# rileyhales/river-route

Measured on AMD Instinct MI355X. Metric: reach-steps/sec, higher is better.
Workload: dtype f64

## Files before the change

river_route_amd/csrc/rr_engine.hip:

```cpp
#include "rr_common.hpp"
#include "rr_kernels_tick.hpp"
#include "rr_kernels_tile.hpp"
#include "rr_kernels_uh.hpp"
#include "rr_kernels_rec.hpp"
#include "rr_kernels_runoff.hpp"
#include "rr_kernels_direct.hpp"
#include "rr_kernels_metrics.hpp"
#include "rr_kernels_overlap.hpp"
#include "rr_kernels_adjoint.hpp"
#include "rr_kernels_adjoint_unit.hpp"
#include "rr_exec.hpp"


extern "C" {

int rr_version(void) { return RR_VERSION_NUM; }

const char *rr_last_error(void) { return g_err.c_str(); }

int rr_device_count(void)
{
    int c = 0;
    if (hipGetDeviceCount(&c) != hipSuccess) return 0;
    return c;
// ... 10 lines not shown
        if (P->ev_last) (void)hipEventDestroy(P->ev_last);
    }
    delete P;
}

int rr_plan_create(int64_t n, const int32_t *csc_indptr, const int32_t *csc_indices, int device, rr_plan **out)
{
    if (!out) return fail(RR_E_INVALID, "rr_plan_create: null out");
    *out = nullptr;
    rr_plan *P = new (std::nothrow) rr_plan();
    if (!P) return fail(RR_E_ALLOC, "rr_plan_create: out of memory");
    if (const char *e = getenv("RR_HW_INPASS")) P->hw_inpass = atoi(e) != 0;
    if (const char *e = getenv("RR_ALLOC_FAIL_AT")) rr::g_dev_fail_in = std::max(0, atoi(e));
    if (const char *e = getenv("RR_WAVE")) { P->wave_enabled = atoi(e) != 0; P->wave_forced = atoi(e) == 1; }
    if (const char *e = getenv("RR_REC_BATCHES")) { P->rec_batches = std::max(1, std::min(kRecMaxLaunchBatches, atoi(e))); P->rec_batches_forced = true; }
    if (const char *e = getenv("RR_WAVE_K")) P->wave_K = std::max(kRec, atoi(e) / kRec * kRec);
    std::string err;
    int rc = rr::build_host_plan(n, csc_indptr, csc_indices, P->h, err);
    if (rc) { delete P; return fail(rc, err); }
    if (device != RR_DEVICE_NONE) {
        int count = rr_device_count(), cus = 0;
        if (device >= 0 && device < count && hipDeviceGetAttribute(&cus, hipDeviceAttributeMultiprocessorCount, device) == hipSuccess && cus > 0) P->cu_count = cus;
    }
    {
        P->wave_threads = kTileThreads;
        int32_t block = P->wave_threads;
        if (const char *e = getenv("RR_TILE_BLOCK")) block = std::max(8, std::min(block, atoi(e)));
        std::vector<int32_t> lag_of((size_t)n);
        for (int64_t i = 0; i < n; ++i) lag_of[i] = P->h.lag[P->h.inv[i]];
        rr::build_tile_plan(P->h.down, lag_of, block, P->tp);
        if (const char *e = getenv("RR_DIRECT")) P->direct_enabled = atoi(e) != 0;
        P->direct_block = block;
        rr::build_direct_plan(P->h.down, lag_of, std::min<int32_t>(kDirectLanes, block), kDirectMaxWindow - 2, block, P->dp);
        P->direct_window = 3;
        for (int32_t sp : P->dp.tile_span) P->direct_window = std::max(P->direct_window, sp + 3);
    }
    if (device != RR_DEVICE_NONE) {
        int count = rr_device_count();
        if (device < 0 || device >= count) {
            delete P;
            return fail(RR_E_NO_DEVICE, "rr_plan_create: HIP device " + std::to_string(device) + " not available (" +
                                            std::to_string(count) + " visible)");
        }
        hipError_t e = hipSetDevice(device);
        if (e != hipSuccess) { delete P; return fail(RR_E_HIP, hipGetErrorString(e)); }
        P->device = device;
        {
            size_t free_b = 0, total_b = 0;
            if (hipMemGetInfo(&free_b, &total_b) == hipSuccess) P->dev_total_bytes = total_b;
        }
        if (const char *e2 = getenv("RR_TILE_LEAN")) P->lean_enabled = atoi(e2) != 0;
        for (int v = 0; v < 7; ++v)
            if (hipFuncSetAttribute((const void *)tile_kernel(v < 4 ? (v & 1) != 0 : v == 5, v < 4 && (v & 2) != 0, v >= 4, v == 6), hipFuncAttributeMaxDynamicSharedMemorySize,
                                    (int)tile_lds_bytes(P->wave_threads)) != hipSuccess) {
                (void)hipGetLastError();
                P->wave_enabled = false;
            }
        for (int v = 0; v < 4; ++v)
            if (hipFuncSetAttribute((const void *)tile_ens_kernel((v & 1) != 0, v >= 2), hipFuncAttributeMaxDynamicSharedMemorySize, (int)tile_lds_bytes(kTileThreads)) != hipSuccess) {
                (void)hipGetLastError();
                P->ens_enabled = false;
            }
        if (const char *e2 = getenv("RR_UH_PAIRS")) P->uh_pairs = atoi(e2) != 0;
        for (int v = 0; v < 4; ++v)
            (void)hipFuncSetAttribute((const void *)rec_in_uh_kernel((v & 1) != 0, 64, 1 + (v >> 1)), hipFuncAttributeMaxDynamicSharedMemorySize, (int)rec_in_uh_lds_bytes(64, 1 + (v >> 1)));
        (void)hipGetLastError();
        const rr::HostPlan &H = P->h;
        const int64_t ni = (int64_t)H.inner_pos.size();
        rc = P->d_child_ptr.alloc(n + 1);
        for (DevBuf<int32_t> *col : {&P->d_lag, &P->d_perm, &P->d_inv}) if (!rc) rc = col->alloc(n);
        if (!rc) rc = P->d_inner_pos.alloc(ni);
        if (!rc) rc = P->d_hwc.alloc(n);
        if (!rc) rc = P->d_bidx.alloc(n);
        if (!rc) rc = P->d_c4_params.alloc(n);
        if (!rc && P->tp.ok) {
            const rr::TilePlan &TP = P->tp;
            const int64_t np = TP.np;
            std::vector<int32_t> inner_idx;
            inner_idx.reserve(ni);
            for (int64_t i = 0; i < n; ++i) if (H.child_ptr[H.inv[i] + 1] > H.child_ptr[H.inv[i]]) inner_idx.push_back((int32_t)i);
            rc = assign(P->d_inner_idx, inner_idx);
            if (!rc) rc = upload_tile_meta(P, TP.lag, TP.xpos, TP.tile_flags);
            if (!rc) rc = assign(P->ts.perm, TP.perm);
            if (!rc) rc = assign(P->d_tinv, TP.inv);
            for (DevBuf<double> *coef : {&P->ts.coef, &P->d_coef_unit, &P->d_coef_hw}) if (!rc) rc = coef->alloc(3 * np);
            if (!rc) rc = P->d_hwcoef.alloc(3 * n);
            if (!rc) rc = P->d_hwq.alloc(n);
            for (DevBuf<double> *state : {&P->ts.sq, &P->ts.ss, &P->ts.si, &P->ts.sqch}) if (!rc) rc = state->alloc(np);
            if (!rc) rc = P->d_full.alloc(n);
            if (!rc) rc = P->d_chan.alloc(n);
        }
        if (!rc) rc = upload_direct_plan(P);
        for (DevBuf<double> *row : {&P->d_w, &P->d_c1row_h, &P->d_c2, &P->d_c3, &P->d_c4}) if (!rc) rc = row->alloc(n);
        if (!rc) rc = P->d_x.alloc(3 * n);
        if (!rc) rc = P->d_isum.alloc(n);
        if (!rc) rc = P->d_qch.alloc(n);
        if (!rc) rc = dev_upload(P->d_child_ptr, H.child_ptr);
        if (!rc) rc = dev_upload(P->d_lag, H.lag);
        if (!rc) rc = dev_upload(P->d_perm, H.perm);
        if (!rc) rc = dev_upload(P->d_inv, H.inv);
        if (!rc) rc = dev_upload(P->d_inner_pos, H.inner_pos);
        if (!rc) rc = dev_upload(P->d_hwc, H.hw_children);
        if (rc) { rr_plan_destroy(P); return rc; }
    }
    *out = P;
    return RR_OK;
}
// ... 1690 lines not shown
```

river_route_amd/csrc/rr_exec.hpp:

```cpp
#pragma once

#include <atomic>

#include "rr_devbuf.hpp"

using rr::DevBuf;


enum class Mode { Rapid, Muskingum, Unit };

struct Rows {
    const double *dev_in = nullptr;
    const float *dev_in32 = nullptr;
    const double *host_in = nullptr;
    int64_t rows_in = 0;
    double *dev_out = nullptr;
    double *host_out = nullptr;
    int64_t rows_out = 0;
    float *dev_out32 = nullptr;
    int64_t out_factor = 1;
    const double *uh_kernel = nullptr, *uh_state = nullptr;
    int64_t uh_nks = 0;
    const RunoffArgs *runoff = nullptr;
    int64_t members = 0, in_pitch = 0, out_pitch = 0;
// ... 612 lines not shown
        if (io.uh_kernel || io.runoff || (!io.dev_out && !io.dev_out32) || (mode == Mode::Unit && (io.dev_in32 || P->n_ghost > 0 || P->n_export > 0)) || nsub > kDirectMaxSub ||
            (io.dev_out32 && (io.out_factor < 1 || (S.KC * kRec) % io.out_factor != 0 || T % io.out_factor != 0)))
            return fail(RR_E_STATE, "route: the direct row path was chosen for a call it does not take");
        const rr::TilePlan &TP = P->dp.skel;
        const int64_t K = S.KC * kRec;
        S.n_tasks = (S.T + K - 1) / K;
        S.n_diags = TP.n_tiles > 0 ? S.n_macro + TP.n_levels - 1 : 0;
        S.n_in_batches = (S.total + 14) / kRecRows + 1;
        S.n_out_batches = TP.np > 0 ? (S.total + kRecRows - 1) / kRecRows : 0;
        for (int32_t i : P->export_reach) {
            if (!P->dp.big[i]) { S.export_lanes = true; continue; }
            S.export_skel = true;
            const int32_t p = TP.inv[i];
            S.export_skew = std::max<int64_t>(S.export_skew, (int64_t)TP.tile_level[TP.tile_of[p]] * S.KS * kRec + (TP.lag[p] & kLagMask));
        }
        DirectArgs &da = S.da;
        da.tiles = P->d_dtiles; da.n_tiles = P->dp.n_tiles; da.lane = P->d_dlane; da.coef = P->d_dcoef; da.q = P->d_dq; da.qch = nullptr;
        if (mode == Mode::Unit) { da.q = P->d_full; da.qch = P->d_chan; }
        da.send_ptr = P->d_dsend_ptr; da.send_lane = P->d_dsend_lane;
        da.in = S.has_in ? io.dev_in : nullptr; da.out = io.dev_out; da.n = n; da.in_rows = (uint32_t)std::max<int64_t>(1, io.rows_in); da.out_rows = (uint32_t)std::max<int64_t>(1, io.rows_out);
        da.in32 = S.has_in ? io.dev_in32 : nullptr; da.out32 = io.dev_out32; da.factor = (int32_t)std::max<int64_t>(1, io.out_factor);
        da.nsub = (int32_t)nsub; da.inv_nsub = 1.0 / (double)nsub;
        da.in32_sel = P->in32_big_endian ? kSelSwap : kSelNative; da.out32_sel = P->out32_big_endian ? kSelSwap : kSelNative;
        da.rec = P->d_ring; da.rec_chunks = (uint32_t)std::max<int64_t>(1, S.rec_chunks); da.np = (int32_t)TP.np;
        da.K = (int32_t)K; da.total = (int32_t)S.T;
        da.exports = export_series; da.n_export = (int32_t)P->n_export;
    }
    if (S.kernel == Kernel::Tile) {
        const rr::TilePlan &TP = P->tp;
        const int64_t K = S.KC * kRec;
        S.n_diags = S.n_macro + TP.n_levels - 1;
        S.n_in_batches = (S.total + 14) / kRecRows + 1;
        S.n_out_batches = (S.total + kRecRows - 1) / kRecRows;
        S.ghost_slack = P->ghost_reach.empty() ? 0 : S.total_ticks + (int64_t)TP.n_levels * K;
        for (int32_t i : P->ghost_reach) { const int32_t p = TP.inv[i]; S.ghost_slack = std::min<int64_t>(S.ghost_slack, (int64_t)TP.tile_level[TP.tile_of[p]] * K + (TP.lag[p] & kLagMask)); }
        for (int32_t i : P->export_reach) { const int32_t p = TP.inv[i]; S.export_skew = std::max<int64_t>(S.export_skew, (int64_t)TP.tile_level[TP.tile_of[p]] * K + (TP.lag[p] & kLagMask)); }
        S.hw = P->hw_inpass && P->lean_enabled && nsub == 1 && S.members == 0 &&
               (mode == Mode::Unit || (mode == Mode::Rapid && !io.runoff && !io.uh_kernel));
        if (S.members > 0) {
            if (S.members > P->ens_cap || (S.rec_chunks * kRec * TP.np) * S.members > P->d_ring.count()) return fail(RR_E_STATE, "route: the ensemble was not reserved");
            if (io.member_coeffs && S.members > P->mc_sets) return fail(RR_E_STATE, "route: fewer coefficient sets than members");
            S.ring_stride = S.rec_chunks * kRec * TP.np;
            S.ta.sq = P->d_esq; S.ta.ss = P->d_ess; S.ta.si = P->d_esi; S.ta.sqch = nullptr;
        }
    }
    if (getenv("RR_VERBOSE") && S.kernel == Kernel::Direct)
        fprintf(stderr, "rr: n=%lld T=%lld direct rows: K=%lld tiles=%d window=%d holes=%lld outlets=%lld; skeleton: positions=%lld tiles=%d levels=%d ring_chunks=%lld (%.1f GB)\n",
                (long long)n, (long long)T, (long long)(S.KC * kRec), P->dp.n_tiles, P->direct_window, (long long)P->dp.n_holes, (long long)P->dp.n_exports,
                (long long)P->dp.skel.np, P->dp.skel.n_tiles, P->dp.skel.n_levels, (long long)S.rec_chunks, (double)S.rec_chunks * kRec * P->dp.skel.np * 8 / 1e9);
    else if (getenv("RR_VERBOSE"))
        fprintf(stderr, "rr: n=%lld T=%lld nsub=%lld tiled=%d K=%lld tiles=%d levels=%d block=%d ghosts=%lld ring_chunks=%lld (%.1f GB) rec_batches=%lld lds=%zu hw_inpass=%d (%lld of %lld headwater positions)\n",
                (long long)n, (long long)T, (long long)nsub, (int)(S.kernel == Kernel::Tile), (long long)(S.KC * kRec), P->tp.n_tiles, P->tp.n_levels, P->tp.block,
                (long long)P->tp.n_ghost, (long long)S.rec_chunks, S.kernel == Kernel::Tile ? (double)S.rec_chunks * kRec * P->tp.np * 8 / 1e9 : 0.0,
                (long long)S.rec_nb, tile_lds_bytes(P->wave_threads), (int)S.hw, (long long)(S.hw ? P->hw_counts[0] : 0), (long long)P->hw_counts[1]);
    if (S.kernel == Kernel::Tick) {
        const int64_t lag_rows = (dmax + nsub - 1) / nsub;
        S.ring_rows = S.in_place ? 0 : std::min<int64_t>(T, lag_rows + 2 * C + 2);
        if (S.ring_rows > 0xFFFFFFFFLL || T > 0x7FFFFFFFLL) return fail(RR_E_INVALID, "route: too many time rows");
        if (S.ring_rows * n > P->d_ring.count() || (!S.in_place && C * n > P->d_mrows.count()) || (host_io && C * n > P->d_stage.count()))
            return fail(RR_E_STATE, "route: work rows of the streaming kernel were not reserved");
        TickArgs &a = S.a;
        a.child_ptr = P->d_child_ptr; a.lag = P->d_lag; a.w = P->d_w; a.c2 = P->d_c2; a.c3 = P->d_c3; a.c4 = P->d_c4;
        a.c1row = P->weights_uniform ? P->d_c1row_h : nullptr;
        a.isum = P->d_isum; a.bidx = P->d_bidx;
        a.ghost = ghost_series; a.exports = export_series; a.n_ghost = (int32_t)P->n_ghost; a.n_export = (int32_t)P->n_export;
        a.total_substeps = S.total; a.nsub = Div32((uint32_t)nsub); a.inv_nsub = 1.0 / (double)nsub;
        if (S.in_place) {
            a.in = io.dev_in; a.in_ld = n; a.in_rows = Div32((uint32_t)std::max<int64_t>(1, io.rows_in));
            a.out = io.dev_out; a.out_ld = n; a.out_rows = Div32((uint32_t)io.rows_out);
        } else {
            a.in = S.has_in ? P->d_ring : nullptr; a.in_ld = n; a.in_rows = Div32((uint32_t)S.ring_rows);
            a.out = P->d_ring; a.out_ld = n; a.out_rows = Div32((uint32_t)S.ring_rows);
        }
    }
    S.max_samples = P->sample_every >= kSampleGroup ? (size_t)std::min<int64_t>(4096, S.total_ticks / P->sample_every + 1) : 0;
    if (S.kernel == Kernel::Tile && S.max_samples > 0) S.max_samples = (size_t)std::min<int64_t>(4096, S.n_diags / 4 + 1);
    if (S.kernel == Kernel::Direct && S.max_samples > 0) S.max_samples = (size_t)std::min<int64_t>(4096, S.n_tasks);
    S.max_samples = std::min(S.max_samples, P->ev.size() / 2);
    if (!P->ev_first) return fail(RR_E_STATE, "route: the plan's events were not reserved");
    HIPCHK(hipEventRecord(P->ev_first, stream));
    return RR_OK;
}

int session_begin(rr_plan *P, Mode mode, int64_t T, int64_t nsub, const Rows &io, hipStream_t stream,
                  const double *ghost_series, double *export_series)
{
    if (P->ses.open) return fail(RR_E_STATE, "a routing call is already open on this plan (rr_stream_end it first)");
    const int rc = session_setup(P, mode, T, nsub, io, stream, ghost_series, export_series);
    P->ses.open = rc == RR_OK;
    return rc;
}

void launch_skel_state_out(const TileSet &ks, double *dst, const DevBuf<double> &state, hipStream_t stream)
{
    if (ks.tp->np > 0) hipLaunchKernelGGL(k_skel_state_out, grid1(ks.tp->np), dim3(kBlock), 0, stream, dst, (const double *)state, ks.perm.get(), ks.pmeta.get(), (int32_t)ks.tp->np);
}

void permute_rows_via(rr_plan *P, int which, const RowView &src, const RowView &dst, int64_t t0, int nrows, double *mrows, hipStream_t stream)
{
    const int64_t n = P->h.n;
    constexpr int E = kPermE;
    const int64_t tile = (int64_t)E * kPermThreads;
    const int rpb = (int)std::max<int64_t>(1, P->perm_rows_per_block);
    dim3 g((unsigned)((n + tile - 1) / tile), (unsigned)((nrows + rpb - 1) / rpb));
    const size_t lds_bytes = (size_t)tile * sizeof(double);
    hipLaunchKernelGGL(k_perm_a<E>, g, dim3(kPermThreads), lds_bytes, stream, src, mrows, n,
                       (const uint16_t *)P->d_slot_a[which], (const int32_t *)P->d_m_index[which], t0, nrows, rpb);
// ... 61 lines not shown

int session_launch_tick(rr_plan *P, int64_t tau)
{
    Session &S = P->ses;
    const int64_t n = P->h.n;
    int64_t p_lo, p_hi;
    if (!tick_window(P->h, tau, S.total, p_lo, p_hi)) return RR_OK;
    TickArgs &a = S.a;
    a.p_lo = (int32_t)p_lo; a.p_hi = (int32_t)p_hi; a.tau = tau;
    a.xc = P->d_x + (tau % 3) * n;
    a.xa = P->d_x + ((tau + 2) % 3) * n;
    a.xb = P->d_x + ((tau + 1) % 3) * n;
    const int64_t phase = S.max_samples > 0 ? P->prof_launches % P->sample_every : -1;
    if (phase == 0 && !S.bracket_open && (size_t)P->prof_brackets < S.max_samples) {
        HIPCHK(hipEventRecord(P->ev[2 * P->prof_brackets], S.stream));
        S.bracket_open = true;
    }
    const dim3 g = grid1(p_hi - p_lo);
    const bool one = S.nsub == 1;
    if (S.mode == Mode::Unit) {
        UnitTickArgs ua{};
        ua.t = a; ua.hw_children = P->d_hwc; ua.qch = P->d_qch;
        ua.a2 = P->unit_general ? P->d_a2 : nullptr; ua.c1own = P->d_c1own;
        if (P->unit_general) { ua.t.c1row = nullptr; ua.zc = P->d_z + (tau % 3) * n; ua.za = P->d_z + ((tau + 2) % 3) * n; }
        hipLaunchKernelGGL(tick_unit_kernel(one), g, dim3(kBlock), 0, S.stream, ua);
    } else {
        hipLaunchKernelGGL(tick_kernel(S.mode == Mode::Rapid, one), g, dim3(kBlock), 0, S.stream, a);
    }
    if (S.bracket_open) {
        S.bracket_reaches += p_hi - p_lo;
        ++P->prof_samples;
        if (P->prof_samples % kSampleGroup == 0) {
            HIPCHK(hipEventRecord(P->ev[2 * P->prof_brackets + 1], S.stream));
            ++P->prof_brackets;
            P->ev_reaches.push_back(S.bracket_reaches);
            S.bracket_reaches = 0;
            S.bracket_open = false;
        }
    }
    ++P->prof_launches;
    return RR_OK;
}

typedef void (*tile_kernel_t)(const TileArgs);

constexpr int kTileThreads = 512;
tile_kernel_t tile_kernel(bool unit, bool sub, bool lean = false, bool nolat = false)
{
    constexpr int T = kTileThreads;
    if (lean && nolat && !unit && !sub) return (tile_kernel_t)k_tile<T, false, false, true, true>;
    return unit ? (sub ? (tile_kernel_t)k_tile<T, true, true> : (lean ? (tile_kernel_t)k_tile<T, true, false, true> : (tile_kernel_t)k_tile<T, true, false>))
                : (sub ? (tile_kernel_t)k_tile<T, false, true> : (lean ? (tile_kernel_t)k_tile<T, false, false, true> : (tile_kernel_t)k_tile<T, false, false>));
}

tile_kernel_t tile_ens_kernel(bool sub, bool mcoef = false)
{
    constexpr int T = kTileThreads;
    if (mcoef) return sub ? (tile_kernel_t)k_tile<T, false, true, false, false, true, true> : (tile_kernel_t)k_tile<T, false, false, false, false, true, true>;
    return sub ? (tile_kernel_t)k_tile<T, false, true, false, false, true> : (tile_kernel_t)k_tile<T, false, false, false, false, true>;
}

int launch_tile_diag(rr_plan *P, const TileSet &ts, TileArgs &w, const double *coef_unit, int64_t d, bool sampled)
{
    Session &S = P->ses;
    const rr::TilePlan &TP = *ts.tp;
    const int64_t l_lo = std::max<int64_t>(0, d - (S.n_macro - 1)), l_hi = std::min<int64_t>(TP.n_levels - 1, d);
    if (l_hi < l_lo) return RR_OK;
    int64_t t_lo = TP.level_start[l_lo], t_hi = TP.level_start[l_hi + 1];
    const int64_t K = (int64_t)w.KC * kRec;
    if (l_lo == 0) {
        const int64_t end0 = TP.level_start[1];
        int64_t hi = std::min<int64_t>(t_hi, end0);
        while (hi > t_lo && (d + 1) * K <= TP.tile_lag_lo[hi - 1]) --hi;
        if (t_hi <= end0) t_hi = hi;
    }
    if (t_hi <= t_lo) return RR_OK;
    w.diag = (int32_t)d; w.t_first = (int32_t)t_lo; w.t_last = (int32_t)t_hi - 1;
    const bool sample = sampled && S.max_samples > 0 && (P->prof_launches % 4) == 0 && (size_t)P->prof_brackets < S.max_samples;
    if (sample) HIPCHK(hipEventRecord(P->ev[2 * P->prof_brackets], S.stream));
    const dim3 g((unsigned)std::min<int64_t>(t_hi - t_lo, (int64_t)P->cu_count * (1024 / P->wave_threads)));
    const size_t lds_bytes = tile_lds_bytes(P->wave_threads);
    const bool unit = S.mode == Mode::Unit;
    const bool lean = S.nsub == 1 && P->lean_enabled;
    if (S.members > 0) {
        const dim3 ge((unsigned)std::min<int64_t>(t_hi - t_lo, std::max<int64_t>(1, ((int64_t)P->cu_count * (1024 / kTileThreads) + S.members - 1) / S.members)), (unsigned)S.members);
        const bool mcoef = S.io.member_coeffs;
        w.tile_filter = 0; w.coef = mcoef ? P->d_mcoef.get() : ts.coef.get();
        hipLaunchKernelGGL(tile_ens_kernel(S.nsub > 1, mcoef), ge, dim3((unsigned)kTileThreads), tile_lds_bytes(kTileThreads), S.stream, w);
    } else {
        w.tile_filter = lean ? 1 : 0;
        w.coef = (lean && unit) ? coef_unit : ts.coef.get();
        const int4 *const pos = w.pos;
        if (lean && S.hw) {
            w.pos = P->d_pmeta_hw;
            if (!unit) w.coef = P->d_coef_hw;
        }
        hipLaunchKernelGGL(tile_kernel(unit, S.nsub > 1, lean, S.mode == Mode::Muskingum), g, dim3((unsigned)P->wave_threads), lds_bytes, S.stream, w);
        w.pos = pos;
        if (lean && ts.n_wide > 0) {
            w.tile_filter = 2; w.coef = ts.coef;
            hipLaunchKernelGGL(tile_kernel(unit, false, false), g, dim3((unsigned)P->wave_threads), lds_bytes, S.stream, w);
        }
    }
    if (sample) {
        HIPCHK(hipEventRecord(P->ev[2 * P->prof_brackets + 1], S.stream));
        int64_t moved = 0;
        for (int64_t c = t_lo; c < t_hi; ++c) {
            const int64_t m = d - TP.tile_level[c];
            if (m < 0 || m >= S.n_macro || m * K >= TP.tile_lag_hi[c] + S.total || (m + 1) * K <= TP.tile_lag_lo[c]) continue;
            moved += TP.tile_ptr[c + 1] - TP.tile_ptr[c];
        }
        P->ev_reaches.push_back(moved * K * std::max<int64_t>(1, S.members));
        P->prof_samples += K;
        ++P->prof_brackets;
    }
    return RR_OK;
}

bool tile_diag_launches(const rr_plan *P, const rr::TilePlan &TP, int64_t d)
{
    const Session &S = P->ses;
    const int64_t l_lo = std::max<int64_t>(0, d - (S.n_macro - 1)), l_hi = std::min<int64_t>(TP.n_levels - 1, d);
    return l_hi >= l_lo && TP.level_start[l_hi + 1] > TP.level_start[l_lo];
}

RecPermArgs rec_args(const rr_plan *P, int64_t batch)
{
    const Session &S = P->ses;
    RecPermArgs ra{};
    ra.in32_sel = P->in32_big_endian ? kSelSwap : kSelNative; ra.out32_sel = P->out32_big_endian ? kSelSwap : kSelNative;
    ra.rec = P->d_ring; ra.rec_chunks = Div32((uint32_t)S.rec_chunks); ra.np = tiles_of(P, S.kernel).tp->np;
    ra.T = S.T; ra.total = S.total; ra.batch = batch; ra.nsub = Div32((uint32_t)S.nsub);
    ra.factor = Div32((uint32_t)std::max<int64_t>(1, S.io.out_factor));
    return ra;
}

void launch_ghost_permute(rr_plan *P, int64_t batch)
{
    Session &S = P->ses;
    RecPermArgs ra = rec_args(P, batch);
    ra.T = S.total; ra.nsub = Div32(1u);
    ra.n = P->n_ghost; ra.colmeta = S.kernel == Kernel::Direct ? P->d_kghostmeta : P->d_ghostmeta;
    ra.rows = RowView{const_cast<double *>(S.ghost_series), P->n_ghost, 0, (uint32_t)S.total};
    hipLaunchKernelGGL(k_rec_in<false>, dim3((unsigned)((P->n_ghost + kRecInCols - 1) / kRecInCols)), dim3(kRecInThreads), 0, rec_stream(P), ra);
}

typedef void (*rec_in_uh_t)(const RecPermArgs, const UhArgs);
constexpr int kUhFusedMaxTaps = 64;
int uh_padded_taps(int64_t n_ks) { return n_ks <= 16 ? 16 : (n_ks <= 48 ? 48 : 64); }
rec_in_uh_t rec_in_uh_kernel(bool sub, int64_t n_ks, int batches, bool in32 = false)
// ... 683 lines not shown
```

river_route_amd/csrc/rr_kernels_tile.hpp:

```cpp
#pragma once

namespace {


struct TileMeta {
    int32_t b0, b1;
    int32_t level;
    int32_t lag_lo, lag_hi;
    int32_t flags;
    int32_t pad0, pad1;
};
constexpr int32_t kTileWide = 1, kTileExports = 2, kTaskTested = 4;
struct TileArgs {
    const TileMeta *tiles;
    const int4 *pos;
    const double *coef;
    double *sq, *ss, *si, *sqch;
    double *exports;
    int32_t n_export;
    double *rec;
    Div32 rec_chunks;
    int32_t np, t_first, t_last, KC, diag, n_macro, total, has_lat;
    int32_t tile_filter;
    Div32 nsub;
// ... 8 lines not shown
constexpr uint32_t kBufferFlags = 0x00020000;
constexpr uint32_t kDropAccess = 0xFFFFFFF0u;
typedef unsigned int u32x2 __attribute__((ext_vector_type(2)));
typedef unsigned int u32x4 __attribute__((ext_vector_type(4)));
__device__ __forceinline__ __amdgpu_buffer_rsrc_t make_rsrc(const void *base, uint32_t bytes)
{
    return __builtin_amdgcn_make_buffer_rsrc(const_cast<void *>(base), 0, (int)bytes, (int)kBufferFlags);
}
__device__ __forceinline__ void store_f64(__amdgpu_buffer_rsrc_t r, uint32_t byte_off, double v)
{
    u32x2 bits;
    __builtin_memcpy(&bits, &v, sizeof bits);
    __builtin_amdgcn_raw_buffer_store_b64(bits, r, (int)byte_off, 0, 0);
}
constexpr int kAuxDefault = 0, kAuxNt = 2;
template <bool NT = false> __device__ __forceinline__ void store_f64x2(__amdgpu_buffer_rsrc_t r, uint32_t byte_off, double2 v)
{
    u32x4 bits;
    __builtin_memcpy(&bits, &v, sizeof bits);
    __builtin_amdgcn_raw_buffer_store_b128(bits, r, (int)byte_off, 0, NT ? kAuxNt : kAuxDefault);
}
template <bool NT = false> __device__ __forceinline__ u32x4 load_b128(__amdgpu_buffer_rsrc_t r, uint32_t byte_off)
{
    return __builtin_amdgcn_raw_buffer_load_b128(r, (int)byte_off, 0, NT ? kAuxNt : kAuxDefault);
}
template <bool NT = false> __device__ __forceinline__ void load_f64x2(__amdgpu_buffer_rsrc_t r, uint32_t byte_off, double &x, double &y)
{
    const u32x4 bits = load_b128<NT>(r, byte_off);
    double2 v;
    __builtin_memcpy(&v, &bits, sizeof v);
    x = v.x; y = v.y;
}

struct TileStreamPolicy {
    bool rec_loads;
    bool rec_stores;
    bool state;
};
constexpr TileStreamPolicy kTileStreams{true, true, false};

__device__ __forceinline__ int32_t fresh(int32_t v) { asm volatile("" : "+v"(v)); return v; }

constexpr int kRec = 16;
constexpr uint32_t kPosBytes = 128u;
__device__ __forceinline__ int64_t rec_elem(uint32_t ring_chunk, int64_t np, int64_t position)
{
    return ((int64_t)ring_chunk * np + position) * kRec;
}
constexpr int kStageLanes = 32;
constexpr int kStageStrideOut = 18;
__device__ __forceinline__ void wave_lds_fence() { asm volatile("s_waitcnt lgkmcnt(0)" ::: "memory"); }
constexpr int kTilePad = 2;
constexpr int kTileAux = 5;
constexpr size_t tile_lds_bytes(int threads)
{
    return (size_t)(2 * ((int64_t)threads + kTilePad) + (threads / 64) * kStageLanes * kStageStrideOut + kTileAux * threads) * sizeof(double);
}

template <int TH, bool UNIT, bool SUB, bool LEAN = false, bool NOLAT = false, bool ENS = false, bool MCOEF = false>
__global__ __launch_bounds__(TH, 4) void k_tile(const TileArgs a)
{
    static_assert(!MCOEF || ENS, "a coefficient set per member: only the member-batched forms");
    extern __shared__ __attribute__((aligned(16))) double lds[];
    const int tid = threadIdx.x;
    const int32_t total = a.total, K = a.KC * kRec;
    constexpr int THP = TH + kTilePad;
    auto stage_of = [&](int32_t t) { return lds + 2 * THP + (size_t)(t >> 6) * (kStageLanes * kStageStrideOut); };
    if (tid < 2) lds[tid * THP + TH] = 0.0;
    auto ring = [&](int32_t chunk) {
        const uint32_t c = a.rec_chunks.mod((uint32_t)chunk);
        return make_rsrc(a.rec + rec_elem(ENS ? c + member_chunk0(a) : c, a.np, 0), (uint32_t)a.np * kPosBytes);
    };

    struct Task { int32_t tile, m, b0, b1, plain; };
    auto select = [&](int32_t from, Task &t) {
        for (int32_t c = from; c >= a.t_first; c -= (int32_t)gridDim.x) {
            const TileMeta tm = a.tiles[c];
            if (a.tile_filter && ((tm.flags & kTileWide) != 0) != (a.tile_filter == 2)) continue;
            const int32_t m = a.diag - tm.level;
            if (m < 0 || m >= a.n_macro) continue;
            if (m * K >= tm.lag_hi + total || (m + 1) * K <= tm.lag_lo) continue;
            t.tile = c; t.m = m; t.b0 = tm.b0; t.b1 = tm.b1;
            t.plain = (tm.flags == 0 && m * K >= tm.lag_hi && (m + 1) * K <= tm.lag_lo + total) ? 1 : (tm.flags | kTaskTested);
            return true;
        }
        return false;
    };
    Task cur;
    if (!select(a.t_last - (int32_t)blockIdx.x, cur)) return;

    double R[kRec], N[kRec];
    auto issue_load = [&](__amdgpu_buffer_rsrc_t src, int32_t b0, int32_t b1, int j, bool real) {
        const int32_t t = fresh(tid), ln = t & 63;
        const int32_t pos = min(b0 + (t - ln) + 8 * j + (ln >> 3), b1 - 1);
        load_f64x2<kTileStreams.rec_loads>(src, real ? (uint32_t)pos * kPosBytes + (uint32_t)((ln & 7) * 16) : kDropAccess, N[2 * j], N[2 * j + 1]);
    };
    auto receive = [&]() {
        const int32_t tl = fresh(tid), lane = tl & 63;
        double *stage = stage_of(tl);
#pragma unroll
        for (int h = 0; h < 2; ++h) {
#pragma unroll
            for (int g = 0; g < 4; ++g)
                reinterpret_cast<double2 *>(stage + (8 * g + (lane >> 3)) * kStageStrideOut)[lane & 7] =
                    make_double2(N[2 * (4 * h + g)], N[2 * (4 * h + g) + 1]);
            wave_lds_fence();
            if (lane / kStageLanes == h) {
                const double2 *src = reinterpret_cast<const double2 *>(stage + (lane % kStageLanes) * kStageStrideOut);
#pragma unroll
                for (int j = 0; j < 8; ++j) { const double2 v = src[j]; R[2 * j] = v.x; R[2 * j + 1] = v.y; }
            }
            wave_lds_fence();
        }
    };

    struct State { int32_t lg, up, xp, uh; double c1, c2, c3, s_prev, qch, isum, q; };
    auto load_state = [&](const Task &t, State &s) {
        s.lg = -1; s.up = 0; s.xp = 0; s.uh = 0;
        s.c1 = s.c2 = s.c3 = s.s_prev = s.qch = s.isum = s.q = 0.0;
        const int32_t p = t.b0 + fresh(tid);
        if (p < t.b1) {
            const int4 pm = a.pos[p];
            const uint32_t cc = (uint32_t)pm.w;
            const int32_t first_up = pm.y - t.b0;
            s.lg = pm.x; s.up = first_up | (int32_t)((cc & 0xFFFFu) << 16);
            s.xp = pm.z;
            if (UNIT) { s.uh = first_up + (int32_t)(cc >> 16); s.qch = stream_load<kTileStreams.state>(a.sqch + p); }
            if (SUB) s.isum = stream_load<kTileStreams.state>(a.si + (ENS ? p + member_pos0(a) : p));
            s.s_prev = stream_load<kTileStreams.state>(a.ss + (ENS ? p + member_pos0(a) : p));
            const double *coef = MCOEF ? a.coef + 3 * (int64_t)member_pos0(a) : a.coef;
            s.q = stream_load<kTileStreams.state>(a.sq + (ENS ? p + member_pos0(a) : p)); s.c1 = coef[3 * (int64_t)p]; s.c2 = coef[3 * (int64_t)p + 1]; s.c3 = coef[3 * (int64_t)p + 2];
        }
    };
    State st;
    load_state(cur, st);
    __amdgpu_buffer_rsrc_t rec_cur = ring(cur.m * a.KC);
#pragma unroll
    for (int j = 0; j < 8; ++j) issue_load(rec_cur, cur.b0, cur.b1, j, true);
    __builtin_amdgcn_s_waitcnt(0x0F70 | 8);
    receive();
    const bool has_lat = a.has_lat != 0;

    for (;;) {
        int32_t lg = LEAN && UNIT ? 0 : st.lg, up = LEAN && UNIT ? 0 : st.up, xp = LEAN && UNIT ? 0 : st.xp, uh = LEAN && UNIT ? 0 : st.uh, sub = 0;
        double c1 = st.c1, c2 = st.c2, c3 = st.c3, s_prev = st.s_prev, qch = st.qch, isum = st.isum;
        const int32_t b0 = cur.b0, tau_begin = cur.m * K;
        lds[(size_t)((tau_begin + 1) & 1) * THP + tid] = st.q;
        constexpr bool kParked = LEAN && UNIT;
        int32_t *const parked = reinterpret_cast<int32_t *>(lds + 2 * THP + (TH / 64) * (kStageLanes * kStageStrideOut));
        if (kParked) {
            double *aux = lds + 2 * THP + (TH / 64) * (kStageLanes * kStageStrideOut);
            reinterpret_cast<int2 *>(parked)[tid] = make_int2(st.up, st.uh);
            reinterpret_cast<int2 *>(parked + 2 * TH)[tid] = make_int2(st.lg, st.xp);
            aux[3 * TH + tid] = st.qch; aux[4 * TH + tid] = st.s_prev;
        }
        auto the_up = [&]() { return kParked ? parked[2 * tid] : fresh(up); };
        auto the_uh = [&]() { return kParked ? parked[2 * tid + 1] : fresh(uh); };
        auto the_lg = [&]() { return kParked ? parked[2 * TH + 2 * tid] : fresh(lg); };
        auto the_xp = [&]() { return kParked ? parked[2 * TH + 2 * tid + 1] : fresh(xp); };
        if (SUB && lg >= 0) {
            const int32_t ts0 = tau_begin - (lg & kLagMask);
            const uint32_t r = a.nsub.mod((uint32_t)(ts0 < 0 ? -ts0 : ts0));
            sub = ts0 >= 0 ? (int32_t)r : (r ? (int32_t)(a.nsub.d - r) : 0);
        }
        Task nxt;
        const bool has_next = select(cur.tile - (int32_t)gridDim.x, nxt);

        auto store_record = [&](__amdgpu_buffer_rsrc_t dst) {
            const int32_t tl = fresh(tid), lane = tl & 63;
            double *stage = stage_of(tl);
#pragma unroll
            for (int h = 0; h < 2; ++h) {
                if (lane / kStageLanes == h) {
                    double2 *mine = reinterpret_cast<double2 *>(stage + (lane % kStageLanes) * kStageStrideOut);
#pragma unroll
                    for (int j = 0; j < 8; ++j) mine[j] = make_double2(R[2 * j], R[2 * j + 1]);
                    int32_t *word = reinterpret_cast<int32_t *>(mine + 8);
                    const int32_t lgw = LEAN ? the_lg() : lg;
                    word[0] = (lgw < 0 || (lgw & (kGhostBit | kTileGhostBit))) ? 1 : 0;
                    if (!SUB) word[1] = (lgw >= 0 && (lgw & kTileExportBit)) ? the_xp() : -1;
                }
                wave_lds_fence();
                const int32_t t = fresh(tid), ln = t & 63;
                const uint32_t first = (uint32_t)(b0 + (t - ln) + h * kStageLanes) * kPosBytes;
// ... 99 lines not shown
                    if (decltype(tested)::value) {
                        const bool active = (uint32_t)(tau0 + s - lagm) < (uint32_t)total;
                        R[s] = active ? qk : R[s];
                        aux_at(3) = active ? r : qc;
                        qk = active ? qk : q_old;
                    } else {
                        R[s] = qk;
                        aux_at(3) = r;
                    }
                    aux_at(4) = s_cur;
                } else {
                    qk = __builtin_fma(c1, s_cur, __builtin_fma(c2, s_prev, __builtin_fma(c3, q_old, (NOLAT && !ghostm) ? 0.0 : R[s])));
                    if (decltype(tested)::value) {
                        const bool active = (uint32_t)(tau0 + s - lagm) < (uint32_t)total;
                        R[s] = active ? qk : R[s];
                        qk = active ? qk : q_old;
                    } else {
                        R[s] = qk;
                    }
                    s_prev = s_cur;
                }
                lds_at(s & 1, own_b) = qk;
                barrier_lds();
            }
        };
        auto store_exports = [&](int32_t tau0, int half) {
            const int32_t lgk = the_lg();
            if (lgk >= 0 && (lgk & kExportBit)) {
                const int32_t ts0 = tau0 + 8 * half - (lgk & kLagMask), slot = the_xp();
#pragma unroll
                for (int s8 = 0; s8 < 8; ++s8)
                    if ((uint32_t)(ts0 + s8) < (uint32_t)total) a.exports[(int64_t)(ts0 + s8) * a.n_export + slot] = R[8 * half + s8];
            }
        };

        barrier_lds();
        for (int32_t cc = 0; cc < a.KC; ++cc) {
            const int32_t chunk = cur.m * a.KC + cc, tau0 = chunk * kRec;
            const bool last = cc + 1 == a.KC;
            const __amdgpu_buffer_rsrc_t rec_next = ring(last ? nxt.m * a.KC : chunk + 1);
            const int32_t nb0 = last ? nxt.b0 : b0, nb1 = last ? nxt.b1 : cur.b1;
            if constexpr (LEAN) {
                const int32_t t = fresh(tid), ln = t & 63, upk = the_up();
                const int32_t cnt = (int32_t)((uint32_t)upk >> 16), u0s = upk & 0xFFFF;
                own_b = t * 8;
                if (NOLAT) { const int32_t lgs = the_lg(); ghostm = lgs >= 0 && (lgs & (kGhostBit | kTileGhostBit)) != 0; }
                if (UNIT) {
                    const int32_t nh = the_uh() - u0s, ni = cnt - nh, i0 = u0s + nh;
                    hw0_b = (nh >= 1 ? u0s : TH) * 8; hw1_b = (nh >= 2 ? u0s + 1 : TH) * 8; hw2_b = (nh >= 3 ? u0s + 2 : TH) * 8;
                    up0_b = (ni >= 1 ? i0 : TH) * 8; up1_b = (ni >= 2 ? i0 + 1 : TH) * 8; up2_b = (ni >= 3 ? i0 + 2 : TH) * 8;
                } else {
                    up0_b = (cnt >= 1 ? u0s : TH) * 8; up1_b = (cnt >= 2 ? u0s + 1 : TH) * 8; up2_b = (cnt >= 3 ? u0s + 2 : TH) * 8;
                }
                const uint32_t nvoff = (uint32_t)(nb0 + (t - ln) + (ln >> 3)) * kPosBytes + (uint32_t)(ln & 7) * 16u;
                const __amdgpu_buffer_rsrc_t src = (!last || has_next) ? rec_next : make_rsrc(a.rec, 0u);
                if (kind == 1) {
                    ticks_plain(std::false_type(), tau0, 0, src, nvoff);
                    ticks_plain(std::false_type(), tau0, 1, src, nvoff);
                } else {
                    { const int32_t lgs = the_lg(); lagm = lgs < 0 ? 0x40000000 : (lgs & kLagMask); }
                    ticks_plain(std::true_type(), tau0, 0, src, nvoff);
                    if (kind & kTileExports) store_exports(tau0, 0);
                    ticks_plain(std::true_type(), tau0, 1, src, nvoff);
                    if (kind & kTileExports) store_exports(tau0, 1);
                }
            } else {
                ticks(tau0, 0, rec_next, nb0, nb1, !last || has_next);
                ticks(tau0, 1, rec_next, nb0, nb1, false);
            }
            store_record(rec_cur);
            if (!LEAN && last && has_next) load_state(nxt, st);
            receive();
            rec_cur = rec_next;
        }
        if ((LEAN ? the_lg() : lg) >= 0) {
            const int32_t p = b0 + tid;
            const double *aux = lds + 2 * THP + (TH / 64) * (kStageLanes * kStageStrideOut);
            constexpr bool kNt = kTileStreams.state;
            stream_store<kNt>(a.sq + (ENS ? p + member_pos0(a) : p), lds[(size_t)((tau_begin + K - 1) & 1) * THP + tid]);
            stream_store<kNt>(a.ss + (ENS ? p + member_pos0(a) : p), (LEAN && UNIT) ? aux[4 * TH + tid] : s_prev);
            if (UNIT) stream_store<kNt>(a.sqch + p, (LEAN && UNIT) ? aux[3 * TH + tid] : qch);
            if (SUB) stream_store<kNt>(a.si + (ENS ? p + member_pos0(a) : p), isum);
        }
        if (LEAN && has_next) load_state(nxt, st);
        if (!has_next) break;
        cur = nxt;
    }
}

__global__ __launch_bounds__(kBlock) void k_tile_state_in(double *sq, double *ss, double *si, const double *q_t, const int32_t *perm,
                                                          const int4 *pos, int32_t np)
{
    const int32_t p = (int32_t)(blockIdx.x * kBlock + threadIdx.x);
    if (p >= np) return;
    double s = 0.0;
    const int4 pm = pos[p];
    const int32_t u0 = pm.y, u1 = u0 + (int32_t)((uint32_t)pm.w & 0xFFFFu);
    for (int32_t u = u0; u < u1; ++u) s += q_t[perm[u]];
    sq[p] = q_t[perm[p]]; ss[p] = s; si[p] = 0.0;
}

__global__ __launch_bounds__(kBlock) void k_tile_unit_state_in(double *sq, double *ss, double *si, double *sqch, const double *full,
                                                               const double *chan, const int32_t *perm, const int4 *pos, int32_t np)
{
    const int32_t p = (int32_t)(blockIdx.x * kBlock + threadIdx.x);
    if (p >= np) return;
    double s = 0.0;
    const int4 pm = pos[p];
    const uint32_t cc = (uint32_t)pm.w;
    const int32_t u0 = pm.y + (int32_t)(cc >> 16), u1 = pm.y + (int32_t)(cc & 0xFFFFu);
    for (int32_t u = u0; u < u1; ++u) s += full[perm[u]];
    sq[p] = full[perm[p]]; ss[p] = s; si[p] = 0.0; sqch[p] = chan[perm[p]];
}

__global__ __launch_bounds__(kBlock) void k_unit_scatter(double *full, double *chan, const double *q_full, const double *q_ch,
                                                         const int32_t *inner_idx, int32_t n_inner)
{
    const int32_t k = (int32_t)(blockIdx.x * kBlock + threadIdx.x);
    if (k >= n_inner) return;
    full[inner_idx[k]] = q_full[k]; chan[inner_idx[k]] = q_ch[k];
}

__global__ __launch_bounds__(kBlock) void k_tile_unit_state_out(double *q_ch, double *q_full, const double *sq, const double *sqch,
                                                                const int32_t *inner_idx, const int32_t *inv, int32_t n_inner)
{
    const int32_t k = (int32_t)(blockIdx.x * kBlock + threadIdx.x);
    if (k >= n_inner) return;
    const int32_t p = inv[inner_idx[k]];
    q_full[k] = sq[p];
    q_ch[k] = sqch[p];
}

__global__ __launch_bounds__(kBlock) void k_unit_gather(double *q_ch, double *q_full, const double *chan, const double *full, const int32_t *inner_idx, int32_t n_inner)
{
    const int32_t k = (int32_t)(blockIdx.x * kBlock + threadIdx.x);
    if (k >= n_inner) return;
    q_full[k] = full[inner_idx[k]]; q_ch[k] = chan[inner_idx[k]];
// ... 36 lines not shown
```

Before: 142.1 billion.

## Prefetch next tile's metadata and state into LDS via global_load_lds DMA

In the lean non-unit non-substep tile kernel, the next task's position metadata, coefficients and q/s state are now fetched asynchronously into a dedicated LDS region with global_load_lds instructions during the last chunk of the current task. At the task boundary it waits and reads them from LDS instead of doing dependent global loads. This hides the load latency between tasks. It also reshapes the LDS budget, replacing the aux area with the staging area for this variant, and adds a microbenchmark that checks the DMA-to-LDS layout.

```diff
diff --git a/profiles/microbench/lds_dma_layout.hip b/profiles/microbench/lds_dma_layout.hip
--- /dev/null
+++ b/profiles/microbench/lds_dma_layout.hip
@@ -0,0 +1,62 @@
+#include <hip/hip_runtime.h>
+#include <cstdint>
+#include <cstdio>
+#include <vector>
+
+template <int BYTES> __device__ __forceinline__ void dma_to_lds(const void *base, uint32_t voff, uint32_t lds_dst)
+{
+    uint32_t keep;
+    if constexpr (BYTES == 16)
+        asm volatile("s_mov_b32 %0, m0\n\ts_mov_b32 m0, %3\n\ts_nop 0\n\tglobal_load_lds_dwordx4 %1, %2\n\ts_mov_b32 m0, %0" : "=&s"(keep) : "v"(voff), "s"(base), "s"(lds_dst) : "memory");
+    else if constexpr (BYTES == 12)
+        asm volatile("s_mov_b32 %0, m0\n\ts_mov_b32 m0, %3\n\ts_nop 0\n\tglobal_load_lds_dwordx3 %1, %2\n\ts_mov_b32 m0, %0" : "=&s"(keep) : "v"(voff), "s"(base), "s"(lds_dst) : "memory");
+    else
+        asm volatile("s_mov_b32 %0, m0\n\ts_mov_b32 m0, %3\n\ts_nop 0\n\tglobal_load_lds_dword %1, %2\n\ts_mov_b32 m0, %0" : "=&s"(keep) : "v"(voff), "s"(base), "s"(lds_dst) : "memory");
+}
+
+constexpr int kDwords = 1024;
+
+template <int BYTES> __global__ __launch_bounds__(128) void probe(const uint32_t *src, uint32_t *out, uint32_t base)
+{
+    extern __shared__ __attribute__((aligned(16))) uint32_t lds[];
+    const int tid = threadIdx.x;
+    for (int i = tid; i < kDwords + (int)base / 4; i += 128) lds[i] = 0xDEADBEEFu;
+    __syncthreads();
+    const uint32_t wave = (uint32_t)__builtin_amdgcn_readfirstlane(tid >> 6);
+    const uint32_t area = (uint32_t)(uintptr_t)(__attribute__((address_space(3))) void *)lds;
+    dma_to_lds<BYTES>(src, (uint32_t)tid * BYTES, area + base + wave * 1024u);
+    asm volatile("s_waitcnt vmcnt(0)\n\ts_waitcnt lgkmcnt(0)\n\ts_barrier" ::: "memory");
+    for (int i = tid; i < kDwords; i += 128) out[i] = lds[base / 4 + i];
+}
+
+template <int BYTES> static int run(const uint32_t *d_src, uint32_t *d_out, uint32_t base)
+{
+    std::vector<uint32_t> h(kDwords);
+    hipLaunchKernelGGL(probe<BYTES>, dim3(1), dim3(128), (kDwords * 4 + base), 0, d_src, d_out, base);
+    if (hipDeviceSynchronize() != hipSuccess || hipMemcpy(h.data(), d_out, kDwords * 4, hipMemcpyDeviceToHost) != hipSuccess) { printf("%d bytes: HIP error\n", BYTES); return 1; }
+    for (int stride : {BYTES, 16}) {
+        std::vector<uint32_t> want(kDwords, 0xDEADBEEFu);
+        for (int l = 0; l < 128; ++l)
+            for (int k = 0; k < BYTES / 4; ++k) want[(l >> 6) * 256 + (l & 63) * stride / 4 + k] = (uint32_t)(l * BYTES / 4 + k);
+        if (want == h) {
+            printf("%2d bytes per lane, base %5u: lane l at base + %d l, nothing else written\n", BYTES, base, stride);
+            return 0;
+        }
+    }
+    printf("%2d bytes per lane, base %5u: neither base + %d l nor base + 16 l:\n", BYTES, base, BYTES);
+    for (int i = 0; i < 160; ++i) printf("%08x%c", h[i], i % 16 == 15 ? '\n' : ' ');
+    return 1;
+}
+
+int main()
+{
+    std::vector<uint32_t> h(4096);
+    for (size_t i = 0; i < h.size(); ++i) h[i] = (uint32_t)i;
+    uint32_t *d_src = nullptr, *d_out = nullptr;
+    if (hipMalloc(&d_src, h.size() * 4) != hipSuccess || hipMalloc(&d_out, kDwords * 4) != hipSuccess) return 2;
+    if (hipMemcpy(d_src, h.data(), h.size() * 4, hipMemcpyHostToDevice) != hipSuccess) return 2;
+    int rc = 0;
+    for (uint32_t base : {0u, 8192u, 20480u}) { rc |= run<16>(d_src, d_out, base); rc |= run<12>(d_src, d_out, base); rc |= run<4>(d_src, d_out, base); }
+    (void)hipFree(d_src); (void)hipFree(d_out);
+    return rc;
+}
diff --git a/river_route_amd/csrc/rr_engine.hip b/river_route_amd/csrc/rr_engine.hip
--- a/river_route_amd/csrc/rr_engine.hip
+++ b/river_route_amd/csrc/rr_engine.hip
@@ -86,7 +86,7 @@
         if (const char *e2 = getenv("RR_TILE_LEAN")) P->lean_enabled = atoi(e2) != 0;
         for (int v = 0; v < 7; ++v)
             if (hipFuncSetAttribute((const void *)tile_kernel(v < 4 ? (v & 1) != 0 : v == 5, v < 4 && (v & 2) != 0, v >= 4, v == 6), hipFuncAttributeMaxDynamicSharedMemorySize,
-                                    (int)tile_lds_bytes(P->wave_threads)) != hipSuccess) {
+                                    (int)tile_kernel_lds_bytes(P->wave_threads, v < 4 ? (v & 1) != 0 : v == 5, v < 4 && (v & 2) != 0, v >= 4)) != hipSuccess) {
                 (void)hipGetLastError();
                 P->wave_enabled = false;
             }
diff --git a/river_route_amd/csrc/rr_exec.hpp b/river_route_amd/csrc/rr_exec.hpp
--- a/river_route_amd/csrc/rr_exec.hpp
+++ b/river_route_amd/csrc/rr_exec.hpp
@@ -688,7 +688,7 @@
         fprintf(stderr, "rr: n=%lld T=%lld nsub=%lld tiled=%d K=%lld tiles=%d levels=%d block=%d ghosts=%lld ring_chunks=%lld (%.1f GB) rec_batches=%lld lds=%zu hw_inpass=%d (%lld of %lld headwater positions)\n",
                 (long long)n, (long long)T, (long long)nsub, (int)(S.kernel == Kernel::Tile), (long long)(S.KC * kRec), P->tp.n_tiles, P->tp.n_levels, P->tp.block,
                 (long long)P->tp.n_ghost, (long long)S.rec_chunks, S.kernel == Kernel::Tile ? (double)S.rec_chunks * kRec * P->tp.np * 8 / 1e9 : 0.0,
-                (long long)S.rec_nb, tile_lds_bytes(P->wave_threads), (int)S.hw, (long long)(S.hw ? P->hw_counts[0] : 0), (long long)P->hw_counts[1]);
+                (long long)S.rec_nb, tile_lds_bytes(P->wave_threads, mode != Mode::Unit && nsub == 1 && P->lean_enabled && S.members == 0), (int)S.hw, (long long)(S.hw ? P->hw_counts[0] : 0), (long long)P->hw_counts[1]);
     if (S.kernel == Kernel::Tick) {
         const int64_t lag_rows = (dmax + nsub - 1) / nsub;
         S.ring_rows = S.in_place ? 0 : std::min<int64_t>(T, lag_rows + 2 * C + 2);
@@ -856,6 +856,8 @@
     return unit ? (sub ? (tile_kernel_t)k_tile<T, true, true> : (lean ? (tile_kernel_t)k_tile<T, true, false, true> : (tile_kernel_t)k_tile<T, true, false>))
                 : (sub ? (tile_kernel_t)k_tile<T, false, true> : (lean ? (tile_kernel_t)k_tile<T, false, false, true> : (tile_kernel_t)k_tile<T, false, false>));
 }
+
+size_t tile_kernel_lds_bytes(int threads, bool unit, bool sub, bool lean) { return tile_lds_bytes(threads, lean && !unit && !sub); }
 
 tile_kernel_t tile_ens_kernel(bool sub, bool mcoef = false)
 {
@@ -899,7 +901,7 @@
             w.pos = P->d_pmeta_hw;
             if (!unit) w.coef = P->d_coef_hw;
         }
-        hipLaunchKernelGGL(tile_kernel(unit, S.nsub > 1, lean, S.mode == Mode::Muskingum), g, dim3((unsigned)P->wave_threads), lds_bytes, S.stream, w);
+        hipLaunchKernelGGL(tile_kernel(unit, S.nsub > 1, lean, S.mode == Mode::Muskingum), g, dim3((unsigned)P->wave_threads), tile_kernel_lds_bytes(P->wave_threads, unit, S.nsub > 1, lean), S.stream, w);
         w.pos = pos;
         if (lean && ts.n_wide > 0) {
             w.tile_filter = 2; w.coef = ts.coef;
diff --git a/river_route_amd/csrc/rr_kernels_tile.hpp b/river_route_amd/csrc/rr_kernels_tile.hpp
--- a/river_route_amd/csrc/rr_kernels_tile.hpp
+++ b/river_route_amd/csrc/rr_kernels_tile.hpp
@@ -84,16 +84,33 @@
 __device__ __forceinline__ void wave_lds_fence() { asm volatile("s_waitcnt lgkmcnt(0)" ::: "memory"); }
 constexpr int kTilePad = 2;
 constexpr int kTileAux = 5;
-constexpr size_t tile_lds_bytes(int threads)
-{
-    return (size_t)(2 * ((int64_t)threads + kTilePad) + (threads / 64) * kStageLanes * kStageStrideOut + kTileAux * threads) * sizeof(double);
+constexpr int kNextPosBytes = 16, kNextCoefBytes = 32, kNextStateBytes = 8;
+constexpr size_t tile_next_bytes(int threads) { return (size_t)threads * (kNextPosBytes + kNextCoefBytes + 2 * kNextStateBytes); }
+constexpr size_t tile_lds_bytes(int threads, bool next_staged = false)
+{
+    return (size_t)(2 * ((int64_t)threads + kTilePad) + (threads / 64) * kStageLanes * kStageStrideOut + (next_staged ? 0 : kTileAux * threads)) * sizeof(double) +
+           (next_staged ? tile_next_bytes(threads) : 0);
+}
+
+template <int BYTES> __device__ __forceinline__ void dma_to_lds(const void *base, uint32_t voff, uint32_t lds_dst)
+{
+    static_assert(BYTES == 4 || BYTES == 12 || BYTES == 16, "global_load_lds: 1, 2, 4, 12 or 16 bytes per lane");
+    uint32_t keep;
+    if constexpr (BYTES == 16)
+        asm volatile("s_mov_b32 %0, m0\n\ts_mov_b32 m0, %3\n\ts_nop 0\n\tglobal_load_lds_dwordx4 %1, %2\n\ts_mov_b32 m0, %0" : "=&s"(keep) : "v"(voff), "s"(base), "s"(lds_dst) : "memory");
+    else if constexpr (BYTES == 12)
+        asm volatile("s_mov_b32 %0, m0\n\ts_mov_b32 m0, %3\n\ts_nop 0\n\tglobal_load_lds_dwordx3 %1, %2\n\ts_mov_b32 m0, %0" : "=&s"(keep) : "v"(voff), "s"(base), "s"(lds_dst) : "memory");
+    else
+        asm volatile("s_mov_b32 %0, m0\n\ts_mov_b32 m0, %3\n\ts_nop 0\n\tglobal_load_lds_dword %1, %2\n\ts_mov_b32 m0, %0" : "=&s"(keep) : "v"(voff), "s"(base), "s"(lds_dst) : "memory");
 }
 
 template <int TH, bool UNIT, bool SUB, bool LEAN = false, bool NOLAT = false, bool ENS = false, bool MCOEF = false>
 __global__ __launch_bounds__(TH, 4) void k_tile(const TileArgs a)
 {
     static_assert(!MCOEF || ENS, "a coefficient set per member: only the member-batched forms");
-    extern __shared__ __attribute__((aligned(16))) double lds[];
+    constexpr bool kTileNextStaged = LEAN && !UNIT && !SUB && !ENS;
+    extern __shared__ __attribute__((aligned(16))) double lds_all[];
+    double *const lds = lds_all + (kTileNextStaged ? tile_next_bytes(TH) / sizeof(double) : 0);
     const int tid = threadIdx.x;
     const int32_t total = a.total, K = a.KC * kRec;
     constexpr int THP = TH + kTilePad;
@@ -162,6 +179,43 @@
             s.s_prev = stream_load<kTileStreams.state>(a.ss + (ENS ? p + member_pos0(a) : p));
             const double *coef = MCOEF ? a.coef + 3 * (int64_t)member_pos0(a) : a.coef;
             s.q = stream_load<kTileStreams.state>(a.sq + (ENS ? p + member_pos0(a) : p)); s.c1 = coef[3 * (int64_t)p]; s.c2 = coef[3 * (int64_t)p + 1]; s.c3 = coef[3 * (int64_t)p + 2];
+        }
+    };
+    constexpr uint32_t kNextCoef = kNextPosBytes * TH, kNextSq = kNextCoef + kNextCoefBytes * TH, kNextSs = kNextSq + kNextStateBytes * TH;
+    auto stage_next = [&](const Task &t) {
+        const int32_t tl = fresh(tid), ln = tl & 63, w0 = t.b0 + (tl - ln), end = t.b1 - 1;
+        const uint32_t wave = (uint32_t)__builtin_amdgcn_readfirstlane(tl >> 6);
+        const uint32_t area = (uint32_t)(uintptr_t)(__attribute__((address_space(3))) void *)lds_all;
+        const uint32_t own = (uint32_t)min(w0 + ln, end);
+        dma_to_lds<16>(a.pos, own * 16u, area + wave * (64u * 16u));
+#pragma unroll
+        for (int h = 0; h < 2; ++h)
+            dma_to_lds<12>(a.coef, own * 24u + (uint32_t)h * 12u, area + kNextCoef + (uint32_t)h * (16u * TH) + wave * (64u * 16u));
+#pragma unroll
+        for (int h = 0; h < 2; ++h) {
+            const int32_t piece = 64 * h + ln, p = min(w0 + (piece >> 1), end);
+            const uint32_t src = (uint32_t)p * (uint32_t)kNextStateBytes + (uint32_t)(piece & 1) * 4u, dst = wave * (64u * kNextStateBytes) + (uint32_t)h * (64u * 4u);
+            dma_to_lds<4>(a.sq, src, area + kNextSq + dst);
+            dma_to_lds<4>(a.ss, src, area + kNextSs + dst);
+        }
+    };
+    auto wait_next = [&]() { __builtin_amdgcn_s_waitcnt(0x0F70 | (16 & 15) | ((16 >> 4) << 14)); };
+    auto read_next = [&](const Task &t, State &s) {
+        barrier_lds();
+        s.lg = -1; s.up = 0; s.xp = 0; s.uh = 0;
+        s.c1 = s.c2 = s.c3 = s.s_prev = s.qch = s.isum = s.q = 0.0;
+        const int32_t tl = fresh(tid);
+        const char *const nx = reinterpret_cast<const char *>(lds_all);
+        if (t.b0 + tl < t.b1) {
+            const int4 pm = reinterpret_cast<const int4 *>(nx)[tl];
+            const uint32_t cc = (uint32_t)pm.w;
+            s.lg = pm.x; s.up = (pm.y - t.b0) | (int32_t)((cc & 0xFFFFu) << 16);
+            s.xp = pm.z;
+            const int4 lo = reinterpret_cast<const int4 *>(nx + kNextCoef)[tl], hi = reinterpret_cast<const int4 *>(nx + kNextCoef + 16 * TH)[tl];
+            const int2 w1 = make_int2(lo.x, lo.y), w2 = make_int2(lo.z, hi.x), w3 = make_int2(hi.y, hi.z);
+            __builtin_memcpy(&s.c1, &w1, 8); __builtin_memcpy(&s.c2, &w2, 8); __builtin_memcpy(&s.c3, &w3, 8);
+            s.q = reinterpret_cast<const double *>(nx + kNextSq)[tl];
+            s.s_prev = reinterpret_cast<const double *>(nx + kNextSs)[tl];
         }
     };
     State st;
@@ -367,6 +421,7 @@
                 } else {
                     up0_b = (cnt >= 1 ? u0s : TH) * 8; up1_b = (cnt >= 2 ? u0s + 1 : TH) * 8; up2_b = (cnt >= 3 ? u0s + 2 : TH) * 8;
                 }
+                if constexpr (kTileNextStaged) { if (last && has_next) stage_next(nxt); }
                 const uint32_t nvoff = (uint32_t)(nb0 + (t - ln) + (ln >> 3)) * kPosBytes + (uint32_t)(ln & 7) * 16u;
                 const __amdgpu_buffer_rsrc_t src = (!last || has_next) ? rec_next : make_rsrc(a.rec, 0u);
                 if (kind == 1) {
@@ -388,6 +443,7 @@
             receive();
             rec_cur = rec_next;
         }
+        if constexpr (kTileNextStaged) wait_next();
         if ((LEAN ? the_lg() : lg) >= 0) {
             const int32_t p = b0 + tid;
             const double *aux = lds + 2 * THP + (TH / 64) * (kStageLanes * kStageStrideOut);
@@ -397,7 +453,7 @@
             if (UNIT) stream_store<kNt>(a.sqch + p, (LEAN && UNIT) ? aux[3 * TH + tid] : qch);
             if (SUB) stream_store<kNt>(a.si + (ENS ? p + member_pos0(a) : p), isum);
         }
-        if (LEAN && has_next) load_state(nxt, st);
+        if (LEAN && has_next) { if constexpr (kTileNextStaged) read_next(nxt, st); else load_state(nxt, st); }
         if (!has_next) break;
         cur = nxt;
     }
```

Result: no change. 142.3 billion (median of 4 runs) (+0.1%).
